# chrished/DEMC.jl

Measured on AMD Instinct MI355X. Metric: chain-updates/sec (N x gens/s) + gens-to-Rhat<1.05, MvNormal d=5 N=1024, higher is better.
Workload: dtype f64

## Files before the change

### demc.jl_amd/csrc/demcz_capi.hip

```cpp
#include "../../include/demcz.h"
#include "demcz_kernels.h"
#include "demcz_kernels_ml.h"
#include "demcz_kernels_pc.h"
#include "demcz_kernels_lr.h"
#include "demcz_kernels_ps.h"
#include "demcz_kernels_ps2.h"
#include "demcz_kernels_ps2d.h"
#include "demcz_pw_dispatch.h"
#include "demcz_mlr_dispatch.h"
#include "demcz_program.h"

#include <rccl/rccl.h>

#include <algorithm>
#include <chrono>
#include <thread>
#include <cstdlib>
#include <deque>
#include <mutex>
#include <cmath>
#include <cstdio>
#include <cstring>
#include <string>
#include <unordered_map>
// ... 119 lines not shown
    bool own_stream = false;
    std::string err;
    std::vector<int32_t> block_offsets, block_indices, slot_of;
    std::vector<double> eps;
    int64_t S = 0;
    int64_t ZS = 0;
    bool full_block = false;
    int ngrp = 1;
    uint64_t gstart = 1ull;
    int mlb_qb = 0;
    double* dZ = nullptr;
    double* dX = nullptr;
    double* dlp = nullptr;
    double* dchain = nullptr;
    double* dchain_alloc = nullptr;
    double* dlogobj = nullptr;
    double* dlp_origin = nullptr;
    bool origin_valid = false;
    double* dtemp = nullptr;
    int64_t temp_cap = 0;
    int32_t* d_block_offsets = nullptr;
    int32_t* d_slot_of = nullptr;
    double* d_eps = nullptr;
    double* d_mu = nullptr;
    double* d_Wp = nullptr;
    double* d_design = nullptr;
    double* d_y = nullptr;
    double* d_scratch = nullptr;
    int64_t scratch_cap = 0;
    double* d_stage = nullptr;
    int64_t stage_cap = 0;
    int64_t M = 0;
    int64_t g_done = 0;
    int64_t g0 = 0;
    int64_t rng_offset = 0;
    bool has_state = false;
    int64_t launches = 0;
    mutable int64_t kernel_counts[1] = {0};
    int last_live = 0, last_ps2 = 0, last_temper = 0, last_dual = 0, last_pw_reg = 0;
    bool external_append = false;
    double* dXprop = nullptr;
    double* dlogu = nullptr;
    bool proposal_pending = false;
    bool gen_open = false;
    double* hc_X = nullptr;
    double* hc_lp = nullptr;
    volatile unsigned int* hc_flag = nullptr;
    unsigned int* hc_count = nullptr;
    unsigned int hc_seq = 0;
    hipStream_t diag_stream = nullptr;
    hipEvent_t diag_ev = nullptr;
    hipEvent_t rhat_side_ev = nullptr;
    bool rhat_side_pending = false;
    double* d_spec_X = nullptr;
    double* d_spec_lp = nullptr;
    hipEvent_t spec_ev = nullptr;
    double* pinned_rhat = nullptr;
    unsigned int* pinned_err = nullptr;
    int64_t pinned_err_launches = -1;
    int64_t pinned_cap = 0;
    bool timing = false;
    std::vector<std::pair<hipEvent_t, hipEvent_t>> timed;
    std::vector<double> series_start_ms, series_dur_ms;
    int64_t timed_launches = 0;
    int64_t live_wg_cap = -1;
    int split_kind = 0;
    int split_lanes = 0;
    int split_per_wg = 1;
    int32_t* d_slot_role = nullptr;
    double* d_rec[2] = {nullptr, nullptr};
    unsigned int* d_live_err = nullptr;
#ifdef DEMCZ_STAMPS
    unsigned long long* d_stamps = nullptr;
#endif
    bool arena = false, rec_in_arena = false, hist_joint = false;
    int64_t arena_gens = 0;
    double* arena_rec[2] = {nullptr, nullptr};
    double* arena_temp = nullptr;
    int64_t rec_cap = 0;
    int rec_cur = 0;
    bool host_paced = false;
    int wpw = 1;
    bool ps_dual = false;
    bool dual_now = false;
    bool lr_spec = false;
    mutable bool lds_raised = false, lds_raised_spec = false;
    bool no_live = false;
    bool live_claimed = false;
    unsigned int live_spin_limit = 0;
    int32_t live_fault_polls = 0;
    int64_t live_fault_g = 0;
    bool in_checked = false;
    struct RunCall { int64_t g_from, g_to; double gamma; bool tempered; std::vector<double> temperature; };
    std::vector<RunCall> live_log;
    double* d_safe_X = nullptr;
    double* d_safe_lp = nullptr;
    bool snap_pending = false;
    int64_t safe_M = 0, safe_M_app = 0, safe_g_done = 0;
    bool replaying = false;
    int32_t live_redos = 0;
    int32_t live_rearms_left = 3;
    int32_t live_rearms = 0;
    int64_t rearm_from = -1;
    uint32_t fail_row_hint = 0xffffffffu;
    struct RecDesc { bool valid = false; int64_t g_first = 0, M = 0, rows = 0; int32_t ngen = 0, boff = 0; } rec_desc[2];
    hipStream_t prod_stream = nullptr;
    hipEvent_t prod_done[2] = {nullptr, nullptr};
    hipEvent_t prod_gate = nullptr;
    bool prod_pending[2] = {false, false};
// ... 285 lines not shown
    if (e != hipSuccess) return e;
    if (n) e = hipMemcpyAsync(*dst, src, n * sizeof(T), hipMemcpyHostToDevice, s);
    return e;
}

static void free_all(demcz_handle* h)
{
    bool drained = !h->comm_dead;
    for (hipStream_t st : {h->stream, h->prod_stream, h->diag_stream, h->comm_stream, h->hs_stream})
        if (st && hipStreamQuery(st) != hipSuccess) drained = false;
    if (h->d_acc) (void)dev_free(h->cfg.device_id, h->d_acc);
    if (h->d_err_all) (void)dev_free(h->cfg.device_id, h->d_err_all);
    if (h->archive_fine) { if (h->dZ) (void)hipFree(h->dZ); h->dZ = nullptr; }
    if (h->pooled_dev) {
        if (h->archive_fine) {
        } else if (drained) {
            g_dev_pool.release(h->dZ, h->cfg.device_id);
        } else {
            g_dev_pool.discard(h->dZ);
        }
        if (h->hist_joint) { if (drained) g_dev_pool.release(h->dchain_alloc, h->cfg.device_id); else g_dev_pool.discard(h->dchain_alloc); }
        h->dZ = nullptr;
        if (h->hist_joint) { h->dchain = nullptr; h->dchain_alloc = nullptr; }
    }
    if (h->hs_stream) stream_release(h->cfg.device_id, h->hs_stream, drained);
    if (drained) { g_host_pool.release(h->hs_chain, -1); g_host_pool.release(h->hs_logobj, -1); }
    else { g_host_pool.discard(h->hs_chain); g_host_pool.discard(h->hs_logobj); }
    void* bufs[] = {h->dZ, h->dX, h->dlp, h->dchain, h->hist_joint ? nullptr : h->dlogobj, h->dlp_origin, h->dtemp, h->d_block_offsets,
                    h->d_slot_of, h->d_slot_role, h->d_eps, h->d_mu, h->d_Wp, h->d_design, h->d_y, h->d_scratch, h->dXprop,
                    h->dlogu, h->d_gather};
    for (void* b : bufs)
        if (b) (void)dev_free(h->cfg.device_id, b);
    for (auto& pe : h->pending) if (pe.ev) (void)hipEventDestroy(pe.ev);
    h->pending.clear();
    for (int b = 0; b < 2; ++b) {
        if (h->d_rec[b] && !h->rec_in_arena) (void)dev_free(h->cfg.device_id, h->d_rec[b]);
        if (b == 0 && h->d_live_err) (void)dev_free(h->cfg.device_id, h->d_live_err);
        if (h->d_send[b]) (void)dev_free(h->cfg.device_id, h->d_send[b]);
        if (h->d_recv[b]) (void)dev_free(h->cfg.device_id, h->d_recv[b]);
        if (h->buf_done[b]) (void)hipEventDestroy(h->buf_done[b]);
    }
    if (h->comm_stream) stream_release(h->cfg.device_id, h->comm_stream, !h->comm_dead && hipStreamQuery(h->comm_stream) == hipSuccess);
    if (h->prod_stream) { if (!h->comm_dead) (void)hipStreamSynchronize(h->prod_stream); stream_release(h->cfg.device_id, h->prod_stream, !h->comm_dead); }
    for (int b = 0; b < 2; ++b) if (h->prod_done[b]) (void)hipEventDestroy(h->prod_done[b]);
    if (h->prod_gate) (void)hipEventDestroy(h->prod_gate);
    if (h->d_stage) (void)host_free(h->d_stage);
    for (auto& pr : h->timed) { (void)hipEventDestroy(pr.first); (void)hipEventDestroy(pr.second); }
    if (h->pinned_rhat) (void)host_free(h->pinned_rhat);
    if (h->pinned_err) (void)host_free(h->pinned_err);
    if (h->d_safe_X) (void)dev_free(h->cfg.device_id, h->d_safe_X);
    if (h->d_safe_lp) (void)dev_free(h->cfg.device_id, h->d_safe_lp);
    if (h->d_spec_X) (void)dev_free(h->cfg.device_id, h->d_spec_X);
    if (h->d_spec_lp) (void)dev_free(h->cfg.device_id, h->d_spec_lp);
    if (h->spec_ev) (void)hipEventDestroy(h->spec_ev);
    if (h->diag_ev) (void)hipEventDestroy(h->diag_ev);
    if (h->rhat_side_ev) (void)hipEventDestroy(h->rhat_side_ev);
    if (h->diag_stream) stream_release(h->cfg.device_id, h->diag_stream, !h->comm_dead && hipStreamQuery(h->diag_stream) == hipSuccess);
    if (h->stall_flag) (void)dev_free(h->cfg.device_id, h->stall_flag);
    if (h->hc_X) (void)hipHostFree(h->hc_X);
    if (h->hc_lp) (void)hipHostFree(h->hc_lp);
    if (h->hc_flag) (void)hipHostFree(const_cast<unsigned int*>(h->hc_flag));
    if (h->hc_count) (void)dev_free(h->cfg.device_id, h->hc_count);
    if (h->xdone) (void)host_free(const_cast<long long*>(h->xdone));
    if (!h->comm_dead) {
        if (h->comm_side) (void)ncclCommDestroy(h->comm_side);
        if (h->comm) (void)ncclCommDestroy(h->comm);
    }
    if (h->own_stream && h->stream) stream_release(h->cfg.device_id, h->stream, !h->comm_dead && hipStreamQuery(h->stream) == hipSuccess);
}

extern "C" int32_t demcz_create(demcz_handle** out, const demcz_config* cfg)
{
    if (!out || !cfg) return fail(nullptr, DEMCZ_ERR_INVALID_ARGUMENT, "demcz_create: null argument");
    *out = nullptr;
    if (cfg->N < 1 || cfg->d < 1 || cfg->d > MAX_D || cfg->K < 1 || cfg->Mcap < 2 || cfg->Gcap < 0 ||
        cfg->Nblocks < 1 || !cfg->block_offsets || !cfg->block_indices || !cfg->eps_scale || cfg->chain_id0 < 0)
        return fail(nullptr, DEMCZ_ERR_INVALID_ARGUMENT,
                    "demcz_create: need N>=1, 1<=d<=64, K>=1, Mcap>=2, Gcap>=0, Nblocks>=1 and block/eps tables");
    if (cfg->lanes_per_chain != 0 && cfg->lanes_per_chain != 1 && cfg->lanes_per_chain != 8 && cfg->lanes_per_chain != 16 &&
        cfg->lanes_per_chain != DEMCZ_LAYOUT_SPLIT && cfg->lanes_per_chain != DEMCZ_LAYOUT_SPLIT_WAVE &&
        cfg->lanes_per_chain != DEMCZ_LAYOUT_PROGRAM_WAVE)
        return fail(nullptr, DEMCZ_ERR_INVALID_ARGUMENT,
                    "demcz_create: lanes_per_chain must be 0 (auto), 1, 8, 16, DEMCZ_LAYOUT_SPLIT, DEMCZ_LAYOUT_SPLIT_WAVE or (program targets) "
                    "DEMCZ_LAYOUT_PROGRAM_WAVE");
    if (cfg->lanes_per_chain == DEMCZ_LAYOUT_PROGRAM_WAVE && cfg->target_kind != DEMCZ_TARGET_PROGRAM)
        return fail(nullptr, DEMCZ_ERR_INVALID_ARGUMENT, "demcz_create: DEMCZ_LAYOUT_PROGRAM_WAVE is the wave-per-chain layout of program targets: "
                                                         "target_kind must be DEMCZ_TARGET_PROGRAM (built-in targets: DEMCZ_LAYOUT_SPLIT_WAVE)");
    const int d = cfg->d;
    if (cfg->block_offsets[0] != 0) return fail(nullptr, DEMCZ_ERR_INVALID_ARGUMENT, "block_offsets[0] must be 0");
    for (int ib = 0; ib < cfg->Nblocks; ++ib) {
        const int a = cfg->block_offsets[ib], b = cfg->block_offsets[ib + 1];
        if (b <= a || b - a > d) return fail(nullptr, DEMCZ_ERR_INVALID_ARGUMENT, "empty or oversized block");
        for (int t = a; t < b; ++t) {
            if (cfg->block_indices[t] < 0 || cfg->block_indices[t] >= d)
                return fail(nullptr, DEMCZ_ERR_INVALID_ARGUMENT, "block index out of range");
            for (int u = a; u < t; ++u)
                if (cfg->block_indices[u] == cfg->block_indices[t])
                    return fail(nullptr, DEMCZ_ERR_INVALID_ARGUMENT, "duplicate index inside a block");
        }
    }
    switch (cfg->target_kind) {
    case DEMCZ_TARGET_MVNORMAL:
        if (!cfg->mu || !cfg->W) return fail(nullptr, DEMCZ_ERR_INVALID_ARGUMENT, "MVNORMAL needs mu and W");
        break;
    case DEMCZ_TARGET_ISO_QUAD:
        if (!cfg->mu) return fail(nullptr, DEMCZ_ERR_INVALID_ARGUMENT, "ISO_QUAD needs mu");
        break;
// ... 2140 lines not shown
    SYNCCHK(h, h->stream);
    return DEMCZ_OK;
}

static int32_t rhat_enqueue(demcz_handle* h, int64_t g_from, int64_t g_to, double* out, bool side = false)
{
    RhatPlan r;
    hipStream_t qs = h->stream;
    static const bool own_env = getenv("DEMCZ_RHAT_OWN_STREAM") != nullptr;
    if (side && !h->comm && !own_env && h->prod_stream) {
        if (!h->diag_ev) HIPCHK(h, hipEventCreateWithFlags(&h->diag_ev, hipEventDisableTiming));
        if (h->after_launch_ev) {
            HIPCHK(h, hipStreamWaitEvent(h->prod_stream, h->after_launch_ev, 0));
        } else {
            HIPCHK(h, hipEventRecord(h->diag_ev, h->stream));
            HIPCHK(h, hipStreamWaitEvent(h->prod_stream, h->diag_ev, 0));
            h->after_launch_ev = h->diag_ev;
        }
        qs = h->prod_stream;
    } else if (side && h->comm && h->peer_mode == 2 && !h->no_live && h->comm_side && h->comm_stream && h->lag == 0) {
        if (!h->diag_ev) HIPCHK(h, hipEventCreateWithFlags(&h->diag_ev, hipEventDisableTiming));
        if (h->after_launch_ev) {
            HIPCHK(h, hipStreamWaitEvent(h->comm_stream, h->after_launch_ev, 0));
        } else {
            HIPCHK(h, hipEventRecord(h->diag_ev, h->stream));
            HIPCHK(h, hipStreamWaitEvent(h->comm_stream, h->diag_ev, 0));
            h->after_launch_ev = h->diag_ev;
        }
        qs = h->comm_stream;
    } else if (side && !h->comm) {
        if (!h->diag_stream) HIPCHK(h, stream_acquire(h->cfg.device_id, &h->diag_stream));
        if (!h->diag_ev) HIPCHK(h, hipEventCreateWithFlags(&h->diag_ev, hipEventDisableTiming));
        if (h->after_launch_ev) {
            HIPCHK(h, hipStreamWaitEvent(h->diag_stream, h->after_launch_ev, 0));
        } else {
            HIPCHK(h, hipEventRecord(h->diag_ev, h->stream));
            HIPCHK(h, hipStreamWaitEvent(h->diag_stream, h->diag_ev, 0));
            h->after_launch_ev = h->diag_ev;
        }
        qs = h->diag_stream;
    }
    if (qs == h->stream && h->rhat_side_pending) {
        HIPCHK(h, hipStreamWaitEvent(h->stream, h->rhat_side_ev, 0));
        h->rhat_side_pending = false;
    }
    struct SideMark {
        demcz_handle* h; hipStream_t qs;
        ~SideMark() {
            if (qs == h->stream) return;
            if (!h->rhat_side_ev && hipEventCreateWithFlags(&h->rhat_side_ev, hipEventDisableTiming) != hipSuccess) { h->rhat_side_ev = nullptr; return; }
            if (hipEventRecord(h->rhat_side_ev, qs) == hipSuccess) h->rhat_side_pending = true;
        }
    } side_mark{h, qs};
    int32_t rc = rhat_prepare(h, g_from, g_to, r, true, qs);
    if (rc) return rc;
    const int d = r.d;
    const int64_t n = r.n;
    const int64_t m = 2 * r.N * h->nranks;
    const bool sharded = (h->comm != nullptr);
    double* sums = r.sums;
    if (!sharded) {
        hipLaunchKernelGGL(rhat_tail_kernel, dim3(d), dim3(256), 0, qs, r.mean_j, r.s2_j, r.N, d, (double)n, (double)m, sums + 3 * d);
        HIPCHK(h, hipGetLastError());
        HIPCHK(h, hipMemcpyAsync(out, sums + 3 * d, (size_t)d * sizeof(double), hipMemcpyDeviceToHost, qs));
        return DEMCZ_OK;
    }
    const ncclComm_t cq = (qs == h->comm_stream && qs != h->stream) ? h->comm_side : h->comm;
    hipLaunchKernelGGL(rhat_reduce_kernel, dim3(d), dim3(256), 0, qs, r.mean_j, r.s2_j, r.N, d, 0, (const double*)nullptr, 1.0, sums);
    HIPCHK(h, hipGetLastError());
    NCCLCHK(h, ncclAllReduce(sums, sums, (size_t)d, ncclDouble, ncclSum, cq, qs));
    hipLaunchKernelGGL(rhat_reduce_kernel, dim3(d), dim3(256), 0, qs, r.mean_j, r.s2_j, r.N, d, 1, (const double*)sums, (double)m, sums + d);
    HIPCHK(h, hipGetLastError());
    NCCLCHK(h, ncclAllReduce(sums + d, sums + d, (size_t)2 * d, ncclDouble, ncclSum, cq, qs));
    hipLaunchKernelGGL(rhat_final_kernel, dim3((unsigned)((d + 63) / 64)), dim3(64), 0, qs, (const double*)(sums + d), d, (double)n, (double)m, sums + 3 * d);
    HIPCHK(h, hipGetLastError());
    HIPCHK(h, hipMemcpyAsync(out, sums + 3 * d, (size_t)d * sizeof(double), hipMemcpyDeviceToHost, qs));
    return DEMCZ_OK;
}

extern "C" int32_t demcz_rhat(demcz_handle* h, int64_t g_from, int64_t g_to, double* rhat)
{
    if (!h || !rhat) return DEMCZ_ERR_INVALID_ARGUMENT;
    int32_t rc = live_verify(h);
    if (rc) return rc;
    rc = rhat_enqueue(h, g_from, g_to, rhat);
    if (rc) return rc;
    SYNCCHK(h, h->stream);
    return DEMCZ_OK;
}

extern "C" int32_t demcz_accept_ratio(demcz_handle* h, int64_t g_from, int64_t g_to, double* ratio)
{
    if (!h || !ratio) return DEMCZ_ERR_INVALID_ARGUMENT;
    int32_t rc = check_hist_range(h, g_from, g_to, "demcz_accept_ratio");
    if (rc) return rc;
    const int64_t N = h->cfg.N, w = g_to - g_from + 1, s0 = g_from - h->g0 - 1;
    if (w < 2) return fail(h, DEMCZ_ERR_INVALID_ARGUMENT, "demcz_accept_ratio: need at least 2 generations");
    HIPCHK(h, hipSetDevice(h->cfg.device_id));
    rc = live_verify(h);
    if (rc) return rc;
    rc = ensure_scratch(h, 2 * N);
    if (rc) return rc;
    {
        const int64_t cb = (N + 63) / 64;
        const int nchunk = (int)std::max<int64_t>(1, std::min<int64_t>(std::min<int64_t>((w - 1 + 31) / 32, 1024), (4096 + cb - 1) / cb));
        unsigned int* cnt = reinterpret_cast<unsigned int*>(h->d_scratch + N);
        HIPCHK(h, hipMemsetAsync(cnt, 0, (size_t)N * sizeof(unsigned int), h->stream));
        hipLaunchKernelGGL(changed_per_chain_kernel, dim3((unsigned)cb, (unsigned)nchunk), dim3(64), 0, h->stream, h->dlogobj, N, s0, w, nchunk, cnt);
        hipLaunchKernelGGL(changed_ratio_kernel, dim3((unsigned)((N + 255) / 256)), dim3(256), 0, h->stream, (const unsigned int*)cnt, N, w, h->d_scratch);
    }
    HIPCHK(h, hipGetLastError());
    HIPCHK(h, hipMemcpyAsync(ratio, h->d_scratch, (size_t)N * sizeof(double), hipMemcpyDeviceToHost, h->stream));
    SYNCCHK(h, h->stream);
// ... 766 lines not shown
        if (hipMemcpy(words, dw, (size_t)n * 16, hipMemcpyDeviceToHost) != hipSuccess ||
            hipMemcpy(normals, dn, (size_t)n * 16, hipMemcpyDeviceToHost) != hipSuccess ||
            hipMemcpy(logu, dl, (size_t)n * 8, hipMemcpyDeviceToHost) != hipSuccess)
            rc = fail(nullptr, DEMCZ_ERR_HIP, "demcz_selftest_draws: kernel or copy failed");
    }
    if (dw) (void)hipFree(dw);
    if (dn) (void)hipFree(dn);
    if (dl) (void)hipFree(dl);
    return rc;
}

#ifdef DEMCZ_STAMPS
extern "C" int32_t demcz_debug_read_stamps(demcz_handle* h, unsigned long long* out, int64_t n_wg)
{
    if (!h || !out || n_wg < 0 || n_wg > DEMCZ_STAMP_WGS || !h->d_stamps) return DEMCZ_ERR_INVALID_ARGUMENT;
    SYNCCHK(h, h->stream);
    HIPCHK(h, hipMemcpy(out, h->d_stamps, (size_t)n_wg * 16 * sizeof(unsigned long long), hipMemcpyDeviceToHost));
    return DEMCZ_OK;
}
#endif

static int32_t run_checked_body(demcz_handle* h, int64_t g_from, int64_t g_to, double gamma, const double* temperature,
                                int64_t every, double threshold, int64_t* g_stop, int32_t* n_checks,
                                double* rhat_max, int32_t n_max, double* rhat_last)
{
    const int d = h->cfg.d;
    int32_t checks = 0;
    int64_t g = g_from;
    if (g_stop) *g_stop = g_to;
    const bool monitor = !(threshold > 0.0);
    const int64_t max_checks = (g_to - g_from + 1) / every + 2;
    HIPCHK(h, hipSetDevice(h->cfg.device_id));
    if (max_checks * d > h->pinned_cap) {
        { int32_t rcq = quiesce_all(h); if (rcq) return rcq; }
        SYNCCHK(h, h->stream);
        if (h->pinned_rhat) (void)host_free(h->pinned_rhat);
        h->pinned_rhat = nullptr; h->pinned_cap = 0;
        const int64_t cap = std::max<int64_t>(max_checks, 1024) * d;
        HIPCHK(h, host_malloc((void**)&h->pinned_rhat, (size_t)cap * sizeof(double)));
        h->pinned_cap = cap;
    }
    double* pinned = h->pinned_rhat;
    auto max_of = [d](const double* r) {
        double mx = r[0];
        for (int p = 1; p < d; ++p) mx = (r[p] > mx || r[p] != r[p]) ? r[p] : mx;
        return mx;
    };
    int32_t rc = DEMCZ_OK;
    const bool speculate = !monitor && !h->comm && h->lag == 0 && !h->external_append && !temperature;
    const int64_t N = h->cfg.N;
    if (speculate) {
        if (!h->d_spec_X) HIPCHK(h, dev_malloc(h->cfg.device_id, (void**)&h->d_spec_X, (size_t)N * d * sizeof(double)));
        if (!h->d_spec_lp) HIPCHK(h, dev_malloc(h->cfg.device_id, (void**)&h->d_spec_lp, (size_t)N * sizeof(double)));
        if (!h->spec_ev) HIPCHK(h, hipEventCreateWithFlags(&h->spec_ev, hipEventDisableTiming));
    }
    bool ahead = false;
    while (g <= g_to && rc == DEMCZ_OK) {
        const int64_t nxt = std::min(g_to, ((g - 1) / every + 1) * every);
        if (!ahead) rc = demcz_run(h, g, nxt, gamma, temperature ? temperature + (g - g_from) : nullptr);
        ahead = false;
        if (rc) break;
        if (nxt % every == 0 && nxt - every >= h->g0) {
            double* slot = pinned + (size_t)checks * d;
            rc = rhat_enqueue(h, nxt - every + 1, nxt, slot, monitor && nxt < g_to);
            if (rc) break;
            ++checks;
            if (!monitor) {
                int64_t M_before = 0;
                if (speculate && nxt < g_to) {
                    if (hipEventRecord(h->spec_ev, h->stream) != hipSuccess) { rc = fail(h, DEMCZ_ERR_HIP, "demcz_run_checked: event failed"); break; }
                    if (hipMemcpyAsync(h->d_spec_X, h->dX, (size_t)N * d * sizeof(double), hipMemcpyDeviceToDevice, h->stream) != hipSuccess ||
                        hipMemcpyAsync(h->d_spec_lp, h->dlp, (size_t)N * sizeof(double), hipMemcpyDeviceToDevice, h->stream) != hipSuccess) {
                        rc = fail(h, DEMCZ_ERR_HIP, "demcz_run_checked: snapshot failed");
                        break;
                    }
                    M_before = h->M_app;
                    const int64_t nn = std::min(g_to, (nxt / every + 1) * every);
                    rc = demcz_run(h, nxt + 1, nn, gamma, nullptr);
                    if (rc) break;
                    ahead = true;
                    if ((rc = sync_event(h, h->spec_ev, "demcz_run_checked")) != DEMCZ_OK) break;
                } else if ((rc = sync_stream(h, h->stream, "demcz_run_checked")) != DEMCZ_OK) {
                    break;
                }
                if (max_of(slot) < threshold) {
                    if (g_stop) *g_stop = nxt;
                    if (ahead) {
                        if ((rc = sync_stream(h, h->stream, "demcz_run_checked")) != DEMCZ_OK) break;
                        rc = check_live_err(h);
                        if (rc) break;
                        if (hipMemcpyAsync(h->dX, h->d_spec_X, (size_t)N * d * sizeof(double), hipMemcpyDeviceToDevice, h->stream) != hipSuccess ||
                            hipMemcpyAsync(h->dlp, h->d_spec_lp, (size_t)N * sizeof(double), hipMemcpyDeviceToDevice, h->stream) != hipSuccess) {
                            rc = fail(h, DEMCZ_ERR_HIP, "demcz_run_checked: restore failed");
                            break;
                        }
                        const size_t rest = (size_t)(h->M_app - M_before) * (size_t)h->ZS;
                        if (rest > 0) {
                            hipLaunchKernelGGL(fill_u64_kernel, dim3((unsigned)((rest + 255) / 256)), dim3(256), 0, h->stream,
                                               reinterpret_cast<unsigned long long*>(h->dZ + (size_t)M_before * h->ZS), rest, LIVE_SENTINEL);
                            if (hipGetLastError() != hipSuccess) { rc = fail(h, DEMCZ_ERR_HIP, "demcz_run_checked: restore failed"); break; }
                        }
                        const int64_t s_lo = nxt - h->g0, s_hi = std::min<int64_t>(h->g_done - h->g0, h->cfg.Gcap);
                        if (s_hi > s_lo &&
                            (hipMemsetAsync(h->dchain + (size_t)N * d * s_lo, 0, (size_t)N * d * (s_hi - s_lo) * sizeof(double), h->stream) != hipSuccess ||
                             hipMemsetAsync(h->dlogobj + (size_t)N * s_lo, 0, (size_t)N * (s_hi - s_lo) * sizeof(double), h->stream) != hipSuccess)) {
                            rc = fail(h, DEMCZ_ERR_HIP, "demcz_run_checked: restore failed");
                            break;
                        }
                        if (h->hs_on) { h->after_launch_ev = nullptr; rc = stream_history(h, nxt + 1, h->g_done); if (rc) break; }
                        h->M_app = M_before;
                        h->M = M_before;
                        h->g_done = nxt;
                        if ((rc = rec_scrub(h)) != DEMCZ_OK) break;
                        if (!h->live_log.empty() && h->live_log.back().g_from == nxt + 1) h->live_log.pop_back();
                        while (!h->acc_log.empty() && h->acc_log.back().g_last > nxt) h->acc_log.pop_back();
                    }
                    break;
                }
            }
        }
        g = nxt + 1;
    }
    h->pinned_err_launches = -1;
    if (rc == DEMCZ_OK && !h->live_log.empty() && h->peer_mode != 2) {
        if (!h->pinned_err && host_malloc((void**)&h->pinned_err, 4 * sizeof(unsigned int)) != hipSuccess) { h->pinned_err = nullptr; (void)hipGetLastError(); }
        if (h->pinned_err && hipMemcpyAsync(h->pinned_err, h->d_live_err, 4 * sizeof(unsigned int), hipMemcpyDeviceToHost, h->stream) == hipSuccess)
            h->pinned_err_launches = h->launches;
    }
    if (rc == DEMCZ_OK) rc = sync_stream(h, h->stream, "demcz_run_checked");
    if (rc == DEMCZ_OK && h->diag_stream) rc = sync_stream(h, h->diag_stream, "demcz_run_checked");
    if (rc == DEMCZ_OK && h->prod_stream) rc = sync_stream(h, h->prod_stream, "demcz_run_checked");
    if (rc == DEMCZ_OK && h->comm_stream) rc = sync_stream(h, h->comm_stream, "demcz_run_checked");
    if (rc == DEMCZ_OK) {
        for (int32_t i = 0; i < checks; ++i)
            if (rhat_max && i < n_max) rhat_max[i] = max_of(pinned + (size_t)i * d);
        if (rhat_last && checks > 0) std::copy(pinned + (size_t)(checks - 1) * d, pinned + (size_t)checks * d, rhat_last);
        if (n_checks) *n_checks = checks;
    }
    return rc;
}

// ... 195 lines not shown
```

### demc.jl_amd/csrc/demcz_kernels.h

```cpp
#pragma once

#include "demcz_device.h"

#pragma clang fp contract(off)

#ifdef DEMCZ_STAMPS
#define DEMCZ_STAMP(P, i) do { if ((P).stamps && threadIdx.x == 0 && blockIdx.x < 65536u) (P).stamps[(size_t)blockIdx.x * 16 + (i)] = __builtin_readcyclecounter(); } while (0)
#else
#define DEMCZ_STAMP(P, i) do { } while (0)
#endif

namespace demcz {

enum { TARGET_MVNORMAL = 0, TARGET_ISO_QUAD = 1, TARGET_LINREG_SSE = 2, TARGET_HOST_CALLBACK = 3, TARGET_PROGRAM = 4 };

constexpr int MAX_D = 64;
constexpr int LINREG_PARTIALS = 16;
constexpr int WINDOW_BS = 64;

struct TargetParams {
    const double* mu;
    const double* Wp;
    double c0;
    const double* design;
// ... 476 lines not shown
}

template <int TARGET>
__global__ void logp_kernel(TargetParams tp, int d, const double* X, int64_t ldX, int64_t n, double* out)
{
    const int64_t c = (int64_t)blockIdx.x * blockDim.x + threadIdx.x;
    if (c >= n) return;
    out[c] = target_logp<TARGET, 0>(tp, d, [&](int j) { return X[c + ldX * j]; });
}

#ifndef DEMCZ_NO_AUX_KERNELS
__global__ void fill_u64_kernel(unsigned long long* p, size_t n, unsigned long long v)
{
    const size_t i = (size_t)blockIdx.x * blockDim.x + threadIdx.x;
    if (i < n) p[i] = v;
}

__global__ void append_rows_kernel(double* Z, int64_t ZS, int64_t M, const double* rows, int64_t nrows,
                                   int64_t ldrows, int d)
{
    const int64_t i = (int64_t)blockIdx.x * blockDim.x + threadIdx.x;
    if (i >= nrows * d) return;
    const int64_t r = i % nrows, p = i / nrows;
    Z[(M + r) * ZS + p] = rows[r + ldrows * p];
}

__global__ void export_rows_kernel(const double* Z, int64_t ZS, int64_t r0, double* out, int64_t nrows, int64_t ldout, int d)
{
    const int64_t i = (int64_t)blockIdx.x * blockDim.x + threadIdx.x;
    if (i >= nrows * d) return;
    const int64_t r = i % nrows, p = i / nrows;
    out[r + ldout * p] = Z[(r0 + r) * ZS + p];
}

__global__ void append_gathered_kernel(double* Z, int64_t ZS, int64_t M, const double* slab, int64_t n_loc,
                                       int R, int d)
{
    const int64_t i = (int64_t)blockIdx.x * blockDim.x + threadIdx.x;
    const int64_t per = n_loc * d;
    if (i >= per * R) return;
    const int64_t r = i / per, rem = i % per, p = rem / n_loc, j = rem % n_loc;
    Z[(M + r * n_loc + j) * ZS + p] = slab[i];
}

__global__ void append_batch_kernel(double* Z, int64_t ZS, int64_t base, const double* slab, int64_t n_loc, int R, int cnt, int d)
{
    const int64_t i = (int64_t)blockIdx.x * blockDim.x + threadIdx.x;
    const int64_t per = n_loc * d;
    if (i >= per * cnt * R) return;
    const int64_t r = i / (per * cnt), rem = i % (per * cnt), sidx = rem / per, rem2 = rem % per, p = rem2 / n_loc, j = rem2 % n_loc;
    Z[(base + (sidx * R + r) * n_loc + j) * ZS + p] = slab[i];
}

__global__ void rhat_moments_kernel(const double* chain, int64_t N, int d, int64_t s0, int64_t n, int nchunk,
                                    double* S1, double* S2)
{
    const int64_t i = (int64_t)blockIdx.x * blockDim.x + threadIdx.x;
    if (i >= N * d) return;
    const int h = blockIdx.y / nchunk, ck = blockIdx.y % nchunk;
    const int64_t per = (n + nchunk - 1) / nchunk;
    const int64_t t0 = ck * per, t1 = (t0 + per < n) ? t0 + per : n;
    const int64_t stride = N * d;
    const double* base = chain + i + stride * (s0 + h * n);
    const double x0 = base[0];
    double a = 0.0, b = 0.0;
    int64_t t = t0;
    for (; t + 8 <= t1; t += 8) {
        double v[8];
#pragma unroll
        for (int u = 0; u < 8; ++u) v[u] = base[stride * (t + u)];
#pragma unroll
        for (int u = 0; u < 8; ++u) {
            const double w = v[u] - x0;
            a += w;
            b = fma(w, w, b);
        }
    }
    for (; t < t1; ++t) {
        double v = base[stride * t] - x0;
        a += v;
        b = fma(v, v, b);
    }
    const int64_t o = i + stride * blockIdx.y;
    S1[o] = a;
    S2[o] = b;
}

__global__ void rhat_chainstats_kernel(const double* chain, int64_t N, int d, int64_t s0, int64_t n, int nchunk,
                                       const double* S1, const double* S2, double* mean_j, double* s2_j)
{
    const int64_t i = (int64_t)blockIdx.x * blockDim.x + threadIdx.x;
    if (i >= N * d) return;
    const int h = blockIdx.y;
    const int64_t stride = N * d;
    const double x0 = chain[i + stride * (s0 + h * n)];
    double a = 0.0, b = 0.0;
    for (int ck = 0; ck < nchunk; ++ck) {
        a += S1[i + stride * (h * nchunk + ck)];
        b += S2[i + stride * (h * nchunk + ck)];
    }
    const double nn = (double)n;
    mean_j[i + stride * h] = x0 + a / nn;
    s2_j[i + stride * h] = (b - a * a / nn) / (nn - 1.0);
}

__global__ void __launch_bounds__(256) rhat_reduce_kernel(const double* mean_j, const double* s2_j, int64_t N, int d,
                                                          int stage, const double* grand, double grand_div, double* out)
{
    __shared__ double ra[256], rb[256];
    const int p = blockIdx.x;
    const int64_t stride = N * d;
    double a = 0.0, b = 0.0;
    const double gm = stage ? grand[p] / grand_div : 0.0;
    int64_t h = 0, c = threadIdx.x;
    while (c >= N) { c -= N; ++h; }
    for (int64_t k = threadIdx.x; k < 2 * N; k += 256) {
        const int64_t at = c + N * p + stride * h;
        const double mj = mean_j[at];
        if (stage == 0) {
            a += mj;
        } else {
            const double dv = mj - gm;
            a = fma(dv, dv, a);
            b += s2_j[at];
        }
        c += 256;
        while (c >= N) { c -= N; ++h; }
    }
    ra[threadIdx.x] = a;
    rb[threadIdx.x] = b;
    __syncthreads();
    for (int s = 128; s > 0; s >>= 1) {
        if ((int)threadIdx.x < s) {
            ra[threadIdx.x] += ra[threadIdx.x + s];
            rb[threadIdx.x] += rb[threadIdx.x + s];
        }
        __syncthreads();
    }
    if (threadIdx.x == 0) {
        out[p] = ra[0];
        if (stage) out[d + p] = rb[0];
    }
}

__global__ void __launch_bounds__(256) rhat_tail_kernel(const double* mean_j, const double* s2_j, int64_t N, int d,
                                                        double n, double m, double* rhat)
{
    __shared__ double ra[256], rb[256];
    const int p = blockIdx.x;
    const int64_t stride = N * d;
    double a = 0.0, b = 0.0;
    int64_t h0 = 0, c0 = threadIdx.x;
    while (c0 >= N) { c0 -= N; ++h0; }
    {
        int64_t h = h0, c = c0;
        for (int64_t k = threadIdx.x; k < 2 * N; k += 256) {
            a += mean_j[c + N * p + stride * h];
            c += 256;
            while (c >= N) { c -= N; ++h; }
        }
    }
    ra[threadIdx.x] = a;
    __syncthreads();
    for (int s = 128; s > 0; s >>= 1) {
        if ((int)threadIdx.x < s) ra[threadIdx.x] += ra[threadIdx.x + s];
        __syncthreads();
    }
    const double gm = ra[0] / m;
    __syncthreads();
    a = 0.0;
    {
        int64_t h = h0, c = c0;
        for (int64_t k = threadIdx.x; k < 2 * N; k += 256) {
            const int64_t at = c + N * p + stride * h;
            const double dv = mean_j[at] - gm;
            a = fma(dv, dv, a);
            b += s2_j[at];
            c += 256;
            while (c >= N) { c -= N; ++h; }
        }
    }
    ra[threadIdx.x] = a;
    rb[threadIdx.x] = b;
    __syncthreads();
    for (int s = 128; s > 0; s >>= 1) {
        if ((int)threadIdx.x < s) {
            ra[threadIdx.x] += ra[threadIdx.x + s];
            rb[threadIdx.x] += rb[threadIdx.x + s];
        }
        __syncthreads();
    }
    if (threadIdx.x == 0) {
        const double B = n / (m - 1.0) * ra[0];
        const double W = rb[0] / m;
        const double varhat = (n - 1.0) / n * W + B / n;
        rhat[p] = sqrt(varhat / W);
    }
}

__global__ void rhat_final_kernel(const double* in, int d, double n, double m, double* rhat)
{
    const int p = blockIdx.x * blockDim.x + threadIdx.x;
    if (p >= d) return;
    const double B = n / (m - 1.0) * in[p];
    const double W = in[d + p] / m;
    const double varhat = (n - 1.0) / n * W + B / n;
    rhat[p] = sqrt(varhat / W);
}

__global__ void __launch_bounds__(256) changed_from_history_kernel(const double* logobj, const double* lp_origin, int64_t N,
                                                                   int64_t s_from, long long* out)
{
    __shared__ int cnt[256];
    const int64_t s = s_from + blockIdx.x;
    const double* cur = logobj + N * s;
    const double* prev = (s == 0) ? lp_origin : logobj + N * (s - 1);
    int k = 0;
    for (int64_t c = threadIdx.x; c < N; c += 256) k += ((cur[c] - prev[c]) != 0.0) ? 1 : 0;
    cnt[threadIdx.x] = k;
    __syncthreads();
    for (int st = 128; st > 0; st >>= 1) {
        if ((int)threadIdx.x < st) cnt[threadIdx.x] += cnt[threadIdx.x + st];
        __syncthreads();
    }
    if (threadIdx.x == 0) out[blockIdx.x] = cnt[0];
}

__global__ void __launch_bounds__(64) changed_per_chain_kernel(const double* logobj, int64_t N, int64_t s0, int64_t w, int nchunk,
                                                               unsigned int* cnt)
{
    const int64_t c = (int64_t)blockIdx.x * 64 + threadIdx.x;
    if (c >= N) return;
    const int64_t per = (w - 1 + nchunk - 1) / nchunk;
    const int64_t t0 = 1 + (int64_t)blockIdx.y * per, t1 = (t0 + per < w) ? t0 + per : w;
    if (t0 >= t1) return;
    unsigned int k = 0;
    double prev = logobj[c + N * (s0 + t0 - 1)];
    for (int64_t t = t0; t < t1; ++t) {
        const double cur = logobj[c + N * (s0 + t)];
        k += ((cur - prev) != 0.0) ? 1u : 0u;
        prev = cur;
    }
    atomicAdd(&cnt[c], k);
}

__global__ void changed_ratio_kernel(const unsigned int* cnt, int64_t N, int64_t w, double* ratio)
{
    const int64_t c = (int64_t)blockIdx.x * blockDim.x + threadIdx.x;
    if (c < N) ratio[c] = (double)cnt[c] / (double)(w - 1);
}

constexpr int MC_TS = 8;
constexpr int MC_VALS = MC_TS * MC_TS + MC_TS;

__global__ void __launch_bounds__(256) meancov_partial_kernel(const double* chain, int64_t N, int d, int64_t s0, int64_t w, int nchunk,
                                                              double* partial)
{
    __shared__ double red[4][MC_VALS];
    const int T = (d + MC_TS - 1) / MC_TS;
    int I = 0, J = (int)blockIdx.z;
// ... 97 lines not shown
```

Baseline: 689.1 million.

## Fuse R-hat moments, chain stats and tail into one last-block-done kernel

After: 683.1 million. About the same (-0.9%).

```diff
diff --git a/demc.jl_amd/csrc/demcz_capi.hip b/demc.jl_amd/csrc/demcz_capi.hip
--- a/demc.jl_amd/csrc/demcz_capi.hip
+++ b/demc.jl_amd/csrc/demcz_capi.hip
@@ -195,9 +195,10 @@
     hipEvent_t diag_ev = nullptr;
     hipEvent_t rhat_side_ev = nullptr;
     bool rhat_side_pending = false;
+    unsigned int* d_rhat_cnt = nullptr;
+    bool rhat_cnt_clean = false;
     double* d_spec_X = nullptr;
     double* d_spec_lp = nullptr;
-    hipEvent_t spec_ev = nullptr;
     double* pinned_rhat = nullptr;
     unsigned int* pinned_err = nullptr;
     int64_t pinned_err_launches = -1;
@@ -589,7 +590,7 @@
     if (h->d_safe_lp) (void)dev_free(h->cfg.device_id, h->d_safe_lp);
     if (h->d_spec_X) (void)dev_free(h->cfg.device_id, h->d_spec_X);
     if (h->d_spec_lp) (void)dev_free(h->cfg.device_id, h->d_spec_lp);
-    if (h->spec_ev) (void)hipEventDestroy(h->spec_ev);
+    if (h->d_rhat_cnt) (void)dev_free(h->cfg.device_id, h->d_rhat_cnt);
     if (h->diag_ev) (void)hipEventDestroy(h->diag_ev);
     if (h->rhat_side_ev) (void)hipEventDestroy(h->rhat_side_ev);
     if (h->diag_stream) stream_release(h->cfg.device_id, h->diag_stream, !h->comm_dead && hipStreamQuery(h->diag_stream) == hipSuccess);
@@ -2836,13 +2837,28 @@
             if (hipEventRecord(h->rhat_side_ev, qs) == hipSuccess) h->rhat_side_pending = true;
         }
     } side_mark{h, qs};
-    int32_t rc = rhat_prepare(h, g_from, g_to, r, true, qs);
+    const bool sharded = (h->comm != nullptr);
+    const bool fused = !sharded && getenv("DEMCZ_NO_FUSED_RHAT") == nullptr;
+    int32_t rc = rhat_prepare(h, g_from, g_to, r, !fused, qs);
     if (rc) return rc;
     const int d = r.d;
     const int64_t n = r.n;
     const int64_t m = 2 * r.N * h->nranks;
-    const bool sharded = (h->comm != nullptr);
     double* sums = r.sums;
+    if (fused) {
+        const unsigned gx = (unsigned)((r.nd + 255) / 256);
+        const size_t cnt_bytes = (((size_t)gx + (size_t)d) * sizeof(unsigned int) + 15) & ~(size_t)15;
+        if (!h->d_rhat_cnt) HIPCHK(h, dev_malloc(h->cfg.device_id, (void**)&h->d_rhat_cnt, cnt_bytes));
+        if (!h->rhat_cnt_clean) HIPCHK(h, hipMemsetAsync(h->d_rhat_cnt, 0, cnt_bytes, qs));
+        h->rhat_cnt_clean = false;
+        double* host_out = (h->pinned_rhat && out >= h->pinned_rhat && out + d <= h->pinned_rhat + h->pinned_cap) ? out : nullptr;
+        hipLaunchKernelGGL(rhat_fused_kernel, dim3(gx, 2 * r.nchunk), dim3(256), 0, qs, h->dchain, r.N, d, r.s0, n, r.nchunk,
+                           r.S1, r.S2, r.mean_j, r.s2_j, (double)m, h->d_rhat_cnt, sums + 3 * d, host_out);
+        HIPCHK(h, hipGetLastError());
+        h->rhat_cnt_clean = true;
+        if (!host_out) HIPCHK(h, hipMemcpyAsync(out, sums + 3 * d, (size_t)d * sizeof(double), hipMemcpyDeviceToHost, qs));
+        return DEMCZ_OK;
+    }
     if (!sharded) {
         hipLaunchKernelGGL(rhat_tail_kernel, dim3(d), dim3(256), 0, qs, r.mean_j, r.s2_j, r.N, d, (double)n, (double)m, sums + 3 * d);
         HIPCHK(h, hipGetLastError());
@@ -3715,7 +3731,6 @@
     if (speculate) {
         if (!h->d_spec_X) HIPCHK(h, dev_malloc(h->cfg.device_id, (void**)&h->d_spec_X, (size_t)N * d * sizeof(double)));
         if (!h->d_spec_lp) HIPCHK(h, dev_malloc(h->cfg.device_id, (void**)&h->d_spec_lp, (size_t)N * sizeof(double)));
-        if (!h->spec_ev) HIPCHK(h, hipEventCreateWithFlags(&h->spec_ev, hipEventDisableTiming));
     }
     bool ahead = false;
     while (g <= g_to && rc == DEMCZ_OK) {
@@ -3725,13 +3740,13 @@
         if (rc) break;
         if (nxt % every == 0 && nxt - every >= h->g0) {
             double* slot = pinned + (size_t)checks * d;
-            rc = rhat_enqueue(h, nxt - every + 1, nxt, slot, monitor && nxt < g_to);
+            rc = rhat_enqueue(h, nxt - every + 1, nxt, slot, (monitor || speculate) && nxt < g_to);
             if (rc) break;
             ++checks;
             if (!monitor) {
                 int64_t M_before = 0;
                 if (speculate && nxt < g_to) {
-                    if (hipEventRecord(h->spec_ev, h->stream) != hipSuccess) { rc = fail(h, DEMCZ_ERR_HIP, "demcz_run_checked: event failed"); break; }
+                    if (!h->rhat_side_pending) { rc = fail(h, DEMCZ_ERR_HIP, "demcz_run_checked: event failed"); break; }
                     if (hipMemcpyAsync(h->d_spec_X, h->dX, (size_t)N * d * sizeof(double), hipMemcpyDeviceToDevice, h->stream) != hipSuccess ||
                         hipMemcpyAsync(h->d_spec_lp, h->dlp, (size_t)N * sizeof(double), hipMemcpyDeviceToDevice, h->stream) != hipSuccess) {
                         rc = fail(h, DEMCZ_ERR_HIP, "demcz_run_checked: snapshot failed");
@@ -3742,7 +3757,7 @@
                     rc = demcz_run(h, nxt + 1, nn, gamma, nullptr);
                     if (rc) break;
                     ahead = true;
-                    if ((rc = sync_event(h, h->spec_ev, "demcz_run_checked")) != DEMCZ_OK) break;
+                    if ((rc = sync_event(h, h->rhat_side_ev, "demcz_run_checked")) != DEMCZ_OK) break;
                 } else if ((rc = sync_stream(h, h->stream, "demcz_run_checked")) != DEMCZ_OK) {
                     break;
                 }
@@ -3750,6 +3765,7 @@
                     if (g_stop) *g_stop = nxt;
                     if (ahead) {
                         if ((rc = sync_stream(h, h->stream, "demcz_run_checked")) != DEMCZ_OK) break;
+                        if (h->prod_stream && (rc = sync_stream(h, h->prod_stream, "demcz_run_checked")) != DEMCZ_OK) break;
                         rc = check_live_err(h);
                         if (rc) break;
                         if (hipMemcpyAsync(h->dX, h->d_spec_X, (size_t)N * d * sizeof(double), hipMemcpyDeviceToDevice, h->stream) != hipSuccess ||
diff --git a/demc.jl_amd/csrc/demcz_kernels.h b/demc.jl_amd/csrc/demcz_kernels.h
--- a/demc.jl_amd/csrc/demcz_kernels.h
+++ b/demc.jl_amd/csrc/demcz_kernels.h
@@ -552,15 +552,12 @@
     Z[(base + (sidx * R + r) * n_loc + j) * ZS + p] = slab[i];
 }
 
-__global__ void rhat_moments_kernel(const double* chain, int64_t N, int d, int64_t s0, int64_t n, int nchunk,
-                                    double* S1, double* S2)
-{
-    const int64_t i = (int64_t)blockIdx.x * blockDim.x + threadIdx.x;
-    if (i >= N * d) return;
-    const int h = blockIdx.y / nchunk, ck = blockIdx.y % nchunk;
+__device__ __forceinline__ void rhat_moments_chunk(const double* chain, int64_t stride, int64_t i, int64_t s0, int64_t n, int nchunk,
+                                                   int y, double* S1, double* S2)
+{
+    const int h = y / nchunk, ck = y % nchunk;
     const int64_t per = (n + nchunk - 1) / nchunk;
     const int64_t t0 = ck * per, t1 = (t0 + per < n) ? t0 + per : n;
-    const int64_t stride = N * d;
     const double* base = chain + i + stride * (s0 + h * n);
     const double x0 = base[0];
     double a = 0.0, b = 0.0;
@@ -581,18 +578,14 @@
         a += v;
         b = fma(v, v, b);
     }
-    const int64_t o = i + stride * blockIdx.y;
+    const int64_t o = i + stride * y;
     S1[o] = a;
     S2[o] = b;
 }
 
-__global__ void rhat_chainstats_kernel(const double* chain, int64_t N, int d, int64_t s0, int64_t n, int nchunk,
-                                       const double* S1, const double* S2, double* mean_j, double* s2_j)
-{
-    const int64_t i = (int64_t)blockIdx.x * blockDim.x + threadIdx.x;
-    if (i >= N * d) return;
-    const int h = blockIdx.y;
-    const int64_t stride = N * d;
+__device__ __forceinline__ void rhat_chainstats_one(const double* chain, int64_t stride, int64_t i, int64_t s0, int64_t n, int nchunk,
+                                                    int h, const double* S1, const double* S2, double* mean_j, double* s2_j)
+{
     const double x0 = chain[i + stride * (s0 + h * n)];
     double a = 0.0, b = 0.0;
     for (int ck = 0; ck < nchunk; ++ck) {
@@ -602,6 +595,30 @@
     const double nn = (double)n;
     mean_j[i + stride * h] = x0 + a / nn;
     s2_j[i + stride * h] = (b - a * a / nn) / (nn - 1.0);
+}
+
+__device__ __forceinline__ double rhat_from_sums(double dev2, double s2, double n, double m)
+{
+    const double B = n / (m - 1.0) * dev2;
+    const double W = s2 / m;
+    const double varhat = (n - 1.0) / n * W + B / n;
+    return sqrt(varhat / W);
+}
+
+__global__ void rhat_moments_kernel(const double* chain, int64_t N, int d, int64_t s0, int64_t n, int nchunk,
+                                    double* S1, double* S2)
+{
+    const int64_t i = (int64_t)blockIdx.x * blockDim.x + threadIdx.x;
+    if (i >= N * d) return;
+    rhat_moments_chunk(chain, N * d, i, s0, n, nchunk, (int)blockIdx.y, S1, S2);
+}
+
+__global__ void rhat_chainstats_kernel(const double* chain, int64_t N, int d, int64_t s0, int64_t n, int nchunk,
+                                       const double* S1, const double* S2, double* mean_j, double* s2_j)
+{
+    const int64_t i = (int64_t)blockIdx.x * blockDim.x + threadIdx.x;
+    if (i >= N * d) return;
+    rhat_chainstats_one(chain, N * d, i, s0, n, nchunk, (int)blockIdx.y, S1, S2, mean_j, s2_j);
 }
 
 __global__ void __launch_bounds__(256) rhat_reduce_kernel(const double* mean_j, const double* s2_j, int64_t N, int d,
@@ -643,11 +660,9 @@
     }
 }
 
-__global__ void __launch_bounds__(256) rhat_tail_kernel(const double* mean_j, const double* s2_j, int64_t N, int d,
-                                                        double n, double m, double* rhat)
-{
-    __shared__ double ra[256], rb[256];
-    const int p = blockIdx.x;
+__device__ __forceinline__ double rhat_tail_param(const double* mean_j, const double* s2_j, int64_t N, int d, int p,
+                                                  double n, double m, double* ra, double* rb)
+{
     const int64_t stride = N * d;
     double a = 0.0, b = 0.0;
     int64_t h0 = 0, c0 = threadIdx.x;
@@ -690,22 +705,85 @@
         }
         __syncthreads();
     }
-    if (threadIdx.x == 0) {
-        const double B = n / (m - 1.0) * ra[0];
-        const double W = rb[0] / m;
-        const double varhat = (n - 1.0) / n * W + B / n;
-        rhat[p] = sqrt(varhat / W);
-    }
+    return rhat_from_sums(ra[0], rb[0], n, m);
+}
+
+__global__ void __launch_bounds__(256) rhat_tail_kernel(const double* mean_j, const double* s2_j, int64_t N, int d,
+                                                        double n, double m, double* rhat)
+{
+    __shared__ double ra[256], rb[256];
+    const double r = rhat_tail_param(mean_j, s2_j, N, d, (int)blockIdx.x, n, m, ra, rb);
+    if (threadIdx.x == 0) rhat[blockIdx.x] = r;
 }
 
 __global__ void rhat_final_kernel(const double* in, int d, double n, double m, double* rhat)
 {
     const int p = blockIdx.x * blockDim.x + threadIdx.x;
     if (p >= d) return;
-    const double B = n / (m - 1.0) * in[p];
-    const double W = in[d + p] / m;
-    const double varhat = (n - 1.0) / n * W + B / n;
-    rhat[p] = sqrt(varhat / W);
+    rhat[p] = rhat_from_sums(in[p], in[d + p], n, m);
+}
+
+__global__ void __launch_bounds__(256) rhat_fused_kernel(const double* chain, int64_t N, int d, int64_t s0, int64_t n, int nchunk,
+                                                         double* S1, double* S2, double* mean_j, double* s2_j, double m,
+                                                         unsigned int* cnt, double* rhat, double* rhat_host)
+{
+    __shared__ double ra[256], rb[256];
+    __shared__ unsigned int elected[256];
+    const int tid = (int)threadIdx.x;
+    const int64_t nd = N * d;
+    const int64_t i = (int64_t)blockIdx.x * 256 + tid;
+    if (i < nd) rhat_moments_chunk(chain, nd, i, s0, n, nchunk, (int)blockIdx.y, S1, S2);
+    asm volatile("s_waitcnt vmcnt(0)" ::: "memory");
+    __syncthreads();
+    if (tid == 0) {
+        __builtin_amdgcn_fence(__ATOMIC_RELEASE, "agent");
+        asm volatile("s_waitcnt vmcnt(0)" ::: "memory");
+        unsigned int* c = cnt + blockIdx.x;
+        const bool last = __hip_atomic_fetch_add(c, 1u, __ATOMIC_RELAXED, __HIP_MEMORY_SCOPE_AGENT) == 2u * (unsigned)nchunk - 1u;
+        if (last) {
+            __hip_atomic_store(c, 0u, __ATOMIC_RELAXED, __HIP_MEMORY_SCOPE_AGENT);
+            __builtin_amdgcn_fence(__ATOMIC_ACQUIRE, "agent");
+            asm volatile("s_waitcnt vmcnt(0)" ::: "memory");
+        }
+        elected[0] = last ? 1u : 0u;
+    }
+    __syncthreads();
+    if (!elected[0]) return;
+    if (i < nd) {
+        rhat_chainstats_one(chain, nd, i, s0, n, nchunk, 0, S1, S2, mean_j, s2_j);
+        rhat_chainstats_one(chain, nd, i, s0, n, nchunk, 1, S1, S2, mean_j, s2_j);
+    }
+    asm volatile("s_waitcnt vmcnt(0)" ::: "memory");
+    __syncthreads();
+    const int64_t i_lo = (int64_t)blockIdx.x * 256, i_hi = (i_lo + 256 < nd ? i_lo + 256 : nd) - 1;
+    const int p_lo = (int)(i_lo / N), np = (int)(i_hi / N) - p_lo + 1;
+    unsigned int* pcnt = cnt + gridDim.x;
+    if (tid < 64) {
+        if (tid == 0) __builtin_amdgcn_fence(__ATOMIC_RELEASE, "agent");
+        asm volatile("s_waitcnt vmcnt(0)" ::: "memory");
+        bool mine = false;
+        for (int q = tid; q < np; q += 64) {
+            const int64_t f = N * (p_lo + q);
+            const unsigned int columns = (unsigned int)((f + N - 1) / 256 - f / 256 + 1);
+            const bool last = __hip_atomic_fetch_add(pcnt + p_lo + q, 1u, __ATOMIC_RELAXED, __HIP_MEMORY_SCOPE_AGENT) == columns - 1u;
+            if (last) __hip_atomic_store(pcnt + p_lo + q, 0u, __ATOMIC_RELAXED, __HIP_MEMORY_SCOPE_AGENT);
+            elected[q] = last ? 1u : 0u;
+            mine = mine || last;
+        }
+        if (__any(mine)) {
+            if (tid == 0) __builtin_amdgcn_fence(__ATOMIC_ACQUIRE, "agent");
+            asm volatile("s_waitcnt vmcnt(0)" ::: "memory");
+        }
+    }
+    __syncthreads();
+    for (int q = 0; q < np; ++q) {
+        if (!elected[q]) continue;
+        const double r = rhat_tail_param(mean_j, s2_j, N, d, p_lo + q, (double)n, m, ra, rb);
+        if (tid == 0) {
+            rhat[p_lo + q] = r;
+            if (rhat_host) rhat_host[p_lo + q] = r;
+        }
+    }
 }
 
 __global__ void __launch_bounds__(256) changed_from_history_kernel(const double* logobj, const double* lp_origin, int64_t N,
```
